# FasterDecoding/TEAL

Hardware: AMD Instinct MI355X
Metric: decode tokens/sec (bs=1), Llama-2-7B fp16 @50% activation sparsity (higher is better)
Workload: dtype f16; 1 GPU; Llama-2-7B bs=1 decode, uniform 50% sparsity, hipGraph-captured step; mode=engine, parallelism=single GPU, context_positions=6..866

## Files before the change

### include/teal_hip.h

```cpp
#ifndef TEAL_HIP_H
#define TEAL_HIP_H

#include <stddef.h>
#include <stdint.h>

#ifdef __cplusplus
extern "C" {
#endif

#define TEAL_OK 0
#define TEAL_ERR_ARG (-1)
#define TEAL_ERR_DTYPE (-2)
#define TEAL_ERR_SHAPE (-3)
#define TEAL_ERR_ALIGN (-4)
#define TEAL_ERR_WORKSPACE (-5)
#define TEAL_ERR_LAUNCH (-6)
#define TEAL_ERR_NO_DEVICE (-7)
#define TEAL_ERR_CONFIG (-8)

#define TEAL_F16 0
#define TEAL_BF16 1

int teal_version(void);
const char* teal_strerror(int code);
// ... 225 lines not shown
#define TEAL_STOP_SEQ 32
#define TEAL_STOP_WORDS 96
#define TEAL_STOP_MAX_IDS 16
#define TEAL_STOP_MAX_SEQS 8
#define TEAL_STOP_MAX_SEQ_LEN 8
#define TEAL_FINISH_RUNNING 0
#define TEAL_FINISH_STOP_TOKEN 1
#define TEAL_FINISH_STOP_SEQUENCE 2
#define TEAL_FINISH_LENGTH 3
#define TEAL_FINISH_CACHE 4
int teal_batched_retire_stops(int32_t* slot_state, const int32_t* tokens, int32_t* pos, const int32_t* history, int history_stride,
                              int32_t* stops, int B, int slot_mask, int max_seq, int count_step, void* stream);


int teal_kv_copy_rows(const void* src_table, const void* dst_table, int n_tensors, int n_heads, int rows, int row_bytes,
                      size_t src_head_stride, size_t dst_head_stride, void* stream);


int teal_cmp_flag_gemv(const void* x, const void* wT, int ld, float* y32, unsigned char* flags, float tau, int Z, int N,
                       int dtype, void* stream);

#ifdef TEAL_DIAGNOSTICS

int teal_set_tuning(int lanes_per_row, int waves, int split, int unroll);

int teal_set_wave_local(int on);

const char* teal_last_launch_desc(void);

int teal_set_fast(int on);

int teal_set_phase_buffer(void* dev_u64);
int teal_set_phase_stride(size_t u64_per_launch);
#endif


int teal_get_config(int Z, int N, int nseg, int* out);

int teal_decode_attention_split_plan(int n_head, int n_kv_head, int head_dim, int max_seq, int nsplit, int roped, int* out);

#ifdef __cplusplus
}
#endif
#endif
```

### teal_amd/_lib.py

```python
from __future__ import annotations

import concurrent.futures
import contextlib
import ctypes
import glob
import os
import shutil
import subprocess
import sys

_PKG = os.path.dirname(os.path.abspath(__file__))
_ROOT = os.path.dirname(_PKG)
CSRC = os.path.join(_PKG, "csrc")
SOURCES = ("teal_kernels.hip", "teal_attention.hip", "teal_sampler.hip", "teal_gemv_w16_f16.hip", "teal_gemv_w16_bf16.hip",
           "teal_gemv_w8_f16.hip", "teal_gemv_w8_bf16.hip", "teal_gemv_fast_f16.hip", "teal_gemv_fast_bf16.hip", "teal_gemv_int4.hip",
           "teal_gemv_fast_w8_f16.hip", "teal_gemv_fast_w8_bf16.hip", "teal_comparators.hip", "teal_prefill.hip",
           "teal_speculative.hip", "teal_batched.hip", "teal_prefix.hip", "teal_logprob.hip", "teal_logit_adjust.hip",
           "teal_sample_rows.hip", "teal_stop.hip")
PRELOAD = {"teal_gemv_fast_f16.hip": 12, "teal_gemv_fast_bf16.hip": 12, "teal_gemv_fast_w8_f16.hip": 12,
           "teal_gemv_fast_w8_bf16.hip": 12, "teal_attention.hip": 12, "teal_sampler.hip": 12}
NO_PACKED_FP32 = ["-Xclang", "-target-feature", "-Xclang", "-packed-fp32-ops"]
FP_CONTRACT = "-ffp-contract=on"
INCLUDE = os.path.join(_ROOT, "include")
OBJ_DIR = os.path.join(CSRC, "_obj")
LIB_PATH = os.path.join(_PKG, "libteal_hip.so")
DIAG_LIB_PATH = os.path.join(_PKG, "libteal_hip_diag.so")
LIB_OVERRIDE = os.environ.get("TEAL_LIB_PATH") or None
OPTIONAL_WITH_OVERRIDE = ("teal_decode_attention_split_roped", "teal_prefill_gemm", "teal_prefill_resid_norm", "teal_prefill_attention",
                          "teal_verify_attention_ws_bytes", "teal_verify_attention", "teal_spec_accept_scratch_bytes", "teal_spec_accept",
                          "teal_batched_sparse_gemm", "teal_batched_round_rows", "teal_batched_decode_attention_ws_bytes",
                          "teal_batched_decode_attention", "teal_batched_sparse_gemm_slots", "teal_batched_decode_attention_slots",
                          "teal_batched_retire", "teal_sample_topk_slot", "teal_kv_copy_rows", "teal_decode_attention_split_plan",
                          "teal_token_logprobs", "teal_score_step", "teal_logit_adjust", "teal_sample_rows",
                          "teal_batched_retire_stops")

EXPORTS = (
    "teal_version", "teal_strerror", "teal_init", "teal_workspace_bytes", "teal_compact",
    "teal_sparse_gemv", "teal_sparse_qkv_gemv", "teal_dense_gemv", "teal_sparse_gateup_silu",
    "teal_get_config", "teal_fused_gemv", "teal_decode_attention", "teal_sample_topk", "teal_sparse_qkv_gemv_ld", "teal_decode_attention_masked", "teal_decode_attention_split", "teal_sparse_qkv_gemv_i8", "teal_decode_attention_split_slabs", "teal_sparse_qkv_gemv_i4",
    "teal_workspace_init", "teal_workspace_release", "teal_sample_topk_ws", "teal_decode_attention_split_ws", "teal_cmp_flag_gemv",
    "teal_decode_attention_split_roped",
    "teal_prefill_gemm", "teal_prefill_resid_norm", "teal_prefill_attention",
    "teal_verify_attention_ws_bytes", "teal_verify_attention", "teal_spec_accept_scratch_bytes", "teal_spec_accept",
    "teal_batched_sparse_gemm", "teal_batched_round_rows", "teal_batched_decode_attention_ws_bytes", "teal_batched_decode_attention",
    "teal_batched_sparse_gemm_slots", "teal_batched_decode_attention_slots", "teal_batched_retire", "teal_sample_topk_slot",
    "teal_kv_copy_rows", "teal_decode_attention_split_plan", "teal_token_logprobs", "teal_score_step",
    "teal_logit_adjust", "teal_sample_rows", "teal_batched_retire_stops",
)

DIAG_EXPORTS = ("teal_set_tuning", "teal_set_fast", "teal_set_wave_local", "teal_set_phase_buffer", "teal_set_phase_stride",
                "teal_last_launch_desc")

_lib = None
_diag = None


def _hipcc() -> str:
    for cand in (os.environ.get("HIPCC"), shutil.which("hipcc"), "/opt/rocm/bin/hipcc"):
        if cand and os.path.exists(cand):
            return cand
    raise RuntimeError("hipcc not found: cannot build libteal_hip.so (no CPU fallback exists)")


def _plan(lib_path: str, obj_dir: str, flags, force: bool, srcs, headers):
    newest_header = max(os.path.getmtime(h) for h in headers)
    hipcc = _hipcc()
    jobs, objs = [], []
    for src in srcs:
        obj = os.path.join(obj_dir, os.path.basename(src)[:-4] + ".o")
        objs.append(obj)
        if not force and os.path.exists(obj) and os.path.getmtime(obj) >= max(os.path.getmtime(src), newest_header):
            continue
        extra = []
        if os.path.basename(src) in PRELOAD:
            extra = ["-mllvm", f"-amdgpu-kernarg-preload-count={PRELOAD[os.path.basename(src)]}"]
        jobs.append(([hipcc, *flags, *extra, "-c", src, "-o", obj], obj))
    return jobs, objs


def build(force: bool = False, verbose: bool = False, out: str | None = None, extra_flags=(), diag: bool = True) -> str:
    headers = glob.glob(os.path.join(CSRC, "*.h")) + [os.path.join(INCLUDE, "teal_hip.h")]
    srcs = [os.path.join(CSRC, f) for f in SOURCES]
    base = ["--offload-arch=gfx950", "-O3", "-std=c++17", "-fPIC", "-Wno-pass-failed", f"-I{INCLUDE}", f"-I{CSRC}", *NO_PACKED_FP32, FP_CONTRACT]
    if out is not None:
# ... 88 lines not shown
        L.teal_batched_round_rows.argtypes = [vp, ci, ci, ci, vp, ci, vp]
        L.teal_batched_decode_attention_ws_bytes.argtypes = [ci, ci, ci]
        L.teal_batched_decode_attention_ws_bytes.restype = sz
        L.teal_batched_decode_attention.argtypes = [vp, ci, vp, vp, vp, vp, vp, vp, sz, ci, ci, ci, ci, ci, ci, vp]
    if hasattr(L, "teal_batched_retire"):
        L.teal_batched_sparse_gemm_slots.argtypes = [vp, vp, vp, ci, ci, vp, ci, ci, vp, sz, ci, ci, vp, vp, ci, ctypes.POINTER(ci), vp]
        L.teal_batched_decode_attention_slots.argtypes = [vp, ci, vp, vp, vp, vp, vp, vp, vp, sz, ci, ci, ci, ci, ci, ci, vp]
        L.teal_batched_retire.argtypes = [vp, vp, vp, ci, ci, ci, ci, vp]
        L.teal_sample_topk_slot.argtypes = [vp, ci, ci, ci, cf, vp, vp, vp, vp, ci, vp, sz, vp, ci, vp]
    if hasattr(L, "teal_kv_copy_rows"):
        L.teal_kv_copy_rows.argtypes = [vp, vp, ci, ci, ci, ci, sz, sz, vp]
    if hasattr(L, "teal_token_logprobs"):
        L.teal_token_logprobs.argtypes = [vp, sz, ci, ci, ci, vp, vp, vp, ci, ci, vp, vp, vp, ci, vp]
        L.teal_score_step.argtypes = [vp, ci, ci, vp, ci, vp, vp, vp, vp]
    if hasattr(L, "teal_logit_adjust"):
        L.teal_logit_adjust.argtypes = [vp, sz, ci, ci, ci, vp, ci, vp, vp, vp, vp, sz, vp, ci, vp]
    if hasattr(L, "teal_sample_rows"):
        L.teal_sample_rows.argtypes = [vp, sz, ci, ci, ci, vp, vp, vp, vp, vp, ci, vp, vp, ci, vp]
    if hasattr(L, "teal_batched_retire_stops"):
        L.teal_batched_retire_stops.argtypes = [vp, vp, vp, vp, ci, vp, ci, ci, ci, ci, vp]
    for name in EXPORTS + (DIAG_EXPORTS if diag else ()):
        if LIB_OVERRIDE and name in OPTIONAL_WITH_OVERRIDE and not hasattr(L, name):
            continue
        getattr(L, name)
        if getattr(L, name).restype is None:
            getattr(L, name).restype = ci
    if diag:
        L.teal_set_tuning.argtypes = [ci, ci, ci, ci]
        L.teal_set_phase_buffer.argtypes = [vp]
        L.teal_set_phase_stride.argtypes = [sz]
        L.teal_set_wave_local.argtypes = [ci]
        L.teal_set_fast.argtypes = [ci]
        L.teal_last_launch_desc.restype = ctypes.c_char_p
    L.teal_is_diagnostics_build = diag
    return L


def load() -> ctypes.CDLL:
    global _lib
    if _lib is None:
        if os.environ.get("TEAL_LIB_FLAVOR", "") == "diag" and not LIB_OVERRIDE:
            _lib = load_diag()
        else:
            _lib = _open(LIB_OVERRIDE or LIB_PATH, False)
    return _lib


def load_diag() -> ctypes.CDLL:
    global _diag
    if _diag is None:
        _diag = _open(DIAG_LIB_PATH, True)
    return _diag


@contextlib.contextmanager
def diagnostics():
    global _lib
    from . import runtime
    prev = load()
    D = load_diag()
    runtime.drop_workspaces()
    _lib = D
    try:
        yield D
    finally:
        D.teal_set_tuning(0, 0, 0, 0)
# ... 13 lines not shown
```

### teal_amd/csrc/teal_attention.hip

```cpp
#include "teal_common.h"

namespace teal {

constexpr int kPhaseRowA = 32;

template <bool BF16, int NT, int HD>
__global__ __launch_bounds__(NT) void decode_attention_kernel(
    const uint16_t* __restrict__ qkv, const uint16_t* __restrict__ rope, const int* __restrict__ pos_ptr,
    uint16_t* __restrict__ k_cache, uint16_t* __restrict__ v_cache, uint16_t* __restrict__ y,
    unsigned long long* __restrict__ mask_out, const float mask_tau,
    const int n_head, const int n_kv, const int max_seq, const float scale, unsigned long long* __restrict__ phase) {
    constexpr int NW = NT / 64;
    constexpr int hd = HD;
    auto stamp_a = [&](const int i) { if (phase && threadIdx.x == 0) phase[(size_t)blockIdx.x * 8 + i] = wall_clock64(); };
    stamp_a(0);
    constexpr int SL = HD / 8;
    constexpr int RW = 64 / SL;
    constexpr int VPF = 256 / (NW * RW) > 0 ? 256 / (NW * RW) : 1;
    extern __shared__ __align__(16) unsigned char smem[];
    float* qs = reinterpret_cast<float*>(smem);
    float* kn = qs + hd;
    float* vn = kn + hd;
    float* red = vn + hd;
    float* part = red + 2 * NW;
// ... 373 lines not shown
#pragma unroll
    for (int w = 0; w < NW; ++w) tot += red[NW + w];
    float o[8];
#pragma unroll
    for (int j = 0; j < 8; ++j) o[j] = 0.0f;
    auto pv_row = [&](const int i, const u32x4 w) {
        const int t = row_of(i);
        if (t >= n) return;
        const float pr = sc[i * STEP + rbase];
        if (!ROPED && t == pos) {
#pragma unroll
            for (int j = 0; j < 8; ++j) o[j] += pr * vn[ds * 8 + j];
        } else {
#pragma unroll
            for (int j = 0; j < 4; ++j) {
                o[2 * j] += pr * bits_to_float(w[j] & 0xFFFFu, BF16);
                o[2 * j + 1] += pr * bits_to_float(w[j] >> 16, BF16);
            }
        }
    };
    if (!rolling) {
#pragma unroll
        for (int i = 0; i < PF; ++i)
            if (i < nsteps) pv_row(i, vreg[i]);
    } else {
        for (int i0 = 0; i0 < nsteps; i0 += RD) {
#pragma unroll
            for (int u = 0; u < RD; ++u) {
                if (i0 + u < nsteps) pv_row(i0 + u, vreg[u]);
                vreg[u] = v_roll(i0 + u + RD);
            }
        }
    }
#pragma unroll
    for (int j = 0; j < 8; ++j) {
        if constexpr (SL <= 8) o[j] = xor_add<8>(o[j]);
        o[j] = xor_add<32>(xor_add<16>(o[j]));
    }
    if (lane < SL) {
#pragma unroll
        for (int j = 0; j < 8; ++j) part[wave * hd + lane * 8 + j] = o[j];
    }
    __syncthreads();
    stamp_p(5);
    if (tid < hd) {
        float acc = 0.0f;
#pragma unroll
        for (int w = 0; w < NW; ++w) acc += part[w * hd + tid];
        out[2 + tid] = acc;
    }
    if (tid == 0) { out[0] = mx; out[1] = tot; }
    stamp_p(7);
}

template <int CTRL>
__device__ __forceinline__ float dpp_lane(const float v) {
    return __builtin_bit_cast(float, __builtin_amdgcn_update_dpp(0, __builtin_bit_cast(int, v), CTRL, 0xf, 0xf, false));
}

template <int NV, int CTRL, int BIT>
__device__ __forceinline__ void fold_level(float* a, const int lane) {
    if constexpr (NV > 1) {
        const bool hi = (lane & BIT) != 0;
#pragma unroll
        for (int k = 0; k < NV / 2; ++k) {
            const float keep = hi ? a[NV / 2 + k] : a[k];
            const float send = hi ? a[k] : a[NV / 2 + k];
            a[k] = keep + dpp_lane<CTRL>(send);
        }
    } else {
        a[0] += dpp_lane<CTRL>(a[0]);
    }
}

template <int REP, int SL>
__device__ __forceinline__ float gqa_reduce_scatter(float* a, const int lane) {
    constexpr int N8 = REP, N4 = (SL == 16 && N8 > 1) ? N8 / 2 : N8, N2 = N4 > 1 ? N4 / 2 : N4, N1 = N2 > 1 ? N2 / 2 : N2;
    static_assert((N1 > 1 ? N1 / 2 : N1) == 1, "more heads than lanes per row");
    if constexpr (SL == 16) fold_level<N8, 0x128, 8>(a, lane);
    fold_level<N4, 0x141, 4>(a, lane);
    fold_level<N2, 0x4E, 2>(a, lane);
    fold_level<N1, 0xB1, 1>(a, lane);
// ... 197 lines not shown
            if (t == pos) w = vnw;
            f32x2 vf[4];
#pragma unroll
            for (int j = 0; j < 4; ++j) vf[j] = (f32x2){bits_to_float(w[j] & 0xFFFFu, BF16), bits_to_float(w[j] >> 16, BF16)};
            float pr[REP];
            const f32x4* pp = reinterpret_cast<const f32x4*>(sc + (size_t)(i * STEP + rbase) * REP);
#pragma unroll
            for (int q4 = 0; q4 < REP / 4; ++q4) {
                const f32x4 pv = pp[q4];
#pragma unroll
                for (int e = 0; e < 4; ++e) pr[q4 * 4 + e] = pv[e];
            }
#pragma unroll
            for (int r = 0; r < REP; ++r) {
                const f32x2 p2 = (f32x2){pr[r], pr[r]};
#pragma unroll
                for (int j = 0; j < 4; ++j) o[r][j] += p2 * vf[j];
            }
        }
    };
    if (nsteps <= PF) {
#pragma unroll
        for (int u = 0; u < PF; ++u)
            if (u < nsteps) v_step(u, vb[u]);
    } else {
        for (int i0 = 0; i0 < nsteps; i0 += RD) {
#pragma unroll
            for (int u = 0; u < RD; ++u) {
                if (i0 + u < nsteps) v_step(i0 + u, vb[u]);
                vb[u] = v_roll(i0 + u + RD);
            }
        }
    }
#pragma unroll
    for (int r = 0; r < REP; ++r)
#pragma unroll
        for (int j = 0; j < 4; ++j)
#pragma unroll
            for (int e = 0; e < 2; ++e) {
                float v = o[r][j][e];
                if constexpr (SL <= 8) v = xor_add<8>(v);
                v = xor_add<32>(xor_add<16>(v));
                o[r][j][e] = v;
            }
    __syncthreads();
    float* part = sc;
    if (lane < SL) {
#pragma unroll
        for (int r = 0; r < REP; ++r)
#pragma unroll
            for (int j = 0; j < 4; ++j)
                *reinterpret_cast<f32x2*>(part + (wave * REP + r) * hd + lane * 8 + 2 * j) = o[r][j];
    }
    __syncthreads();
    for (int c = tid; c < REP * hd; c += NT) {
        float acc = 0.0f;
#pragma unroll
        for (int w = 0; w < NW; ++w) acc += part[w * REP * hd + c];
        out_of(c / hd)[2 + (c % hd)] = acc;
    }
    if (tid < REP) {
        float tot = 0.0f;
#pragma unroll
        for (int w = 0; w < NW; ++w) tot += red[(REP + tid) * NW + w];
        float m = red[tid * NW];
#pragma unroll
        for (int w = 1; w < NW; ++w) m = fmaxf(m, red[tid * NW + w]);
        out_of(tid)[0] = m;
        out_of(tid)[1] = tot;
    }
}

template <bool BF16>
__global__ __launch_bounds__(128) void decode_attention_merge_kernel(const float* __restrict__ partials,
                                                                     uint16_t* __restrict__ y,
                                                                     unsigned long long* __restrict__ mask_out,
                                                                     const float mask_tau, const int hd, const int nsplit) {
    const int h = blockIdx.x, tid = threadIdx.x;
    if (tid >= hd) return;
    merge_head<BF16>(partials + (size_t)h * nsplit * (hd + 2), y + (size_t)h * hd,
                            mask_out ? mask_out + ((size_t)h * hd >> 6) : nullptr, mask_tau, hd, nsplit, tid, tid & 63);
}

constexpr int kGqaMinSeq8 = 2048;
constexpr int kGqaMinSeq = 4096;
constexpr size_t kGqaMaxLds = 128 * 1024;
constexpr size_t kSplitMaxLds = 64 * 1024;

inline bool split_shape_ok(const int n_head, const int n_kv_head, const int head_dim, const int max_seq, const int nsplit) {
    return (head_dim == 64 || head_dim == 128) && n_head > 0 && n_kv_head > 0 && n_head % n_kv_head == 0 && max_seq > 0 &&
           nsplit >= 1 && nsplit <= 64;
// ... 186 lines not shown
```

### teal_amd/csrc/teal_common.h

```cpp
#pragma once
#include <hip/hip_runtime.h>

#include <math.h>
#include <stdint.h>

#include <type_traits>

#include "teal_hip.h"

namespace teal {


typedef uint32_t u32x4 __attribute__((ext_vector_type(4)));
typedef uint32_t u32x2 __attribute__((ext_vector_type(2)));
typedef _Float16 f16x2 __attribute__((ext_vector_type(2)));

constexpr int kMaxSeg = 3;
constexpr int kMaxSplit = 32;


struct Seg {
    const void* w;
    void* y;
    float tau;
// ... 155 lines not shown
    const int t0 = __builtin_amdgcn_readlane(v, 15);
    const int t1 = __builtin_amdgcn_readlane(v, 31);
    const int t2 = __builtin_amdgcn_readlane(v, 47);
    return v + (lane >= 16 ? t0 : 0) + (lane >= 32 ? t1 : 0) + (lane >= 48 ? t2 : 0);
}

__device__ __forceinline__ float wave_sum_f(float v) {
    auto shr = [](float a, auto ctrl) {
        return __builtin_bit_cast(float, __builtin_amdgcn_update_dpp(0, __builtin_bit_cast(int, a), decltype(ctrl)::value, 0xf, 0xf, false));
    };
    v += shr(v, std::integral_constant<int, 0x111>{});
    v += shr(v, std::integral_constant<int, 0x112>{});
    v += shr(v, std::integral_constant<int, 0x114>{});
    v += shr(v, std::integral_constant<int, 0x118>{});
    const int iv = __builtin_bit_cast(int, v);
    return __builtin_bit_cast(float, __builtin_amdgcn_readlane(iv, 15)) +
           __builtin_bit_cast(float, __builtin_amdgcn_readlane(iv, 31)) +
           __builtin_bit_cast(float, __builtin_amdgcn_readlane(iv, 47)) +
           __builtin_bit_cast(float, __builtin_amdgcn_readlane(iv, 63));
}

template <int OFF>
__device__ __forceinline__ float xor_add(const float v) {
    const int iv = __builtin_bit_cast(int, v);
    if constexpr (OFF == 8) {
        return v + __builtin_bit_cast(float, __builtin_amdgcn_update_dpp(iv, iv, 0x128, 0xf, 0xf, false));
    } else if constexpr (OFF == 16) {
        return v + __builtin_bit_cast(float, __builtin_amdgcn_ds_swizzle(iv, 0x401F));
    } else {
        return v + __shfl_xor(v, OFF);
    }
}

__device__ __forceinline__ float wave_max_f(float v) {
    auto shr = [](float a, auto ctrl) {
        return __builtin_bit_cast(float, __builtin_amdgcn_update_dpp(__builtin_bit_cast(int, a), __builtin_bit_cast(int, a), decltype(ctrl)::value, 0xf, 0xf, false));
    };
    v = fmaxf(v, shr(v, std::integral_constant<int, 0x111>{}));
    v = fmaxf(v, shr(v, std::integral_constant<int, 0x112>{}));
    v = fmaxf(v, shr(v, std::integral_constant<int, 0x114>{}));
    v = fmaxf(v, shr(v, std::integral_constant<int, 0x118>{}));
    const int iv = __builtin_bit_cast(int, v);
    return fmaxf(fmaxf(__builtin_bit_cast(float, __builtin_amdgcn_readlane(iv, 15)), __builtin_bit_cast(float, __builtin_amdgcn_readlane(iv, 31))),
                 fmaxf(__builtin_bit_cast(float, __builtin_amdgcn_readlane(iv, 47)), __builtin_bit_cast(float, __builtin_amdgcn_readlane(iv, 63))));
}

template <int SL>
__device__ __forceinline__ float row_slices_sum(float v) {
    if constexpr (SL == 16) {
        auto ror = [](float a, auto ctrl) {
            return __builtin_bit_cast(float, __builtin_amdgcn_update_dpp(0, __builtin_bit_cast(int, a), decltype(ctrl)::value, 0xf, 0xf, false));
        };
        v += ror(v, std::integral_constant<int, 0x128>{});
        v += ror(v, std::integral_constant<int, 0x124>{});
        v += ror(v, std::integral_constant<int, 0x122>{});
        v += ror(v, std::integral_constant<int, 0x121>{});
        return v;
    } else {
#pragma unroll
        for (int d = 1; d < SL; d <<= 1) v += __shfl_xor(v, d);
        return v;
    }
}


__device__ __forceinline__ int lane_rank(unsigned long long mask) {
// ... 41 lines not shown
```

### teal_amd/csrc/teal_gemv_fast.h

```cpp
#pragma once
#include "teal_gemv_fast_decl.h"
#include "teal_gemv_kernel.h"

namespace teal {

#define TEAL_FAST_ARGS_BATCH(a)                                                                                         \
    asm volatile("" ::"s"((a).w0), "s"((a).w1), "s"((a).y), "s"((a).ws), "s"((a).mask_out), "s"((a).resid_out),          \
                 "s"((a).phase), "s"((a).ticket), "s"((a).ld0), "s"((a).ld1), "s"((a).seg_tile1), "s"((a).seg_tile2), "s"((a).tau0),       \
                 "s"((a).tau1), "s"((a).tau2), "s"((a).mask_tau), "s"((a).ws_stride), "s"((a).att_hd), "s"((a).att_ns),  \
                 "s"((a).cap), "s"((a).w1_tile), "s"((a).scale0), "s"((a).scale1), "s"((a).sum32))


template <bool BF16, int MODE, bool PAIR, int LPR, int KR, bool EXACT, bool PHASE, int U = 4, bool W8 = false, bool ROPE = false>
__global__ __launch_bounds__(1024) void gemv_fast_kernel(const void* in0, const void* in1, const void* in2,
                                                         const int* row_index, const int Z, const int nslabs,
                                                         const float eps, const int split_p, const FastArgs a) {
    static_assert(!(W8 && PAIR), "int8 gate|up runs unpaired (two images of 128-byte row segments)");
    static_assert(!ROPE || (MODE == 1 && !PAIR && !W8), "the RoPE / KV-append epilogue belongs to the fused wqkv projection");
    constexpr int WAVES = 16;
    constexpr int RPW = 64 / LPR;
    constexpr int CPL = 8;
    constexpr int BN = LPR * CPL;
    constexpr int WB = W8 ? 1 : 2;
    using wvec = std::conditional_t<W8, u32x2, u32x4>;
// ... 315 lines not shown
            consume(wa, w2a, xa);
            if constexpr (PHASE) { if (!first_done) { first_done = true; stamp(4); } }
            eb = ebn;
            if (!fb) break;
            ebn = eb + STEP;
            fa = full(ebn);
            if (fa) issue(wa, w2a, xa, ebn);
            consume(wbb, w2b, xb);
            eb = ebn;
        }
        if (eb < nloc) {
#pragma unroll
            for (int u = 0; u < U; ++u) {
                const int e = eb + u * RPW + g;
                const bool ok = e < nloc;
                const uint32_t ent = list[ok ? e : nloc - 1];
                xa[u] = ok ? bits_to_float(ent & 0xFFFFu, BF16) : 0.0f;
                wvec t = __builtin_nontemporal_load(reinterpret_cast<const wvec*>(wp + (size_t)(ent >> 16) * ldb));
                if (!ok) t = wvec(0u);
                wa[u] = t;
                if constexpr (PAIR) {
                    wvec t2 = __builtin_nontemporal_load(reinterpret_cast<const wvec*>(wp2 + (size_t)(ent >> 16) * ldb2));
                    if (!ok) t2 = wvec(0u);
                    w2a[u] = t2;
                }
            }
            consume(wa, w2a, xa);
        }
    }
    stamp(5);
    if (prio_set) __builtin_amdgcn_s_setprio(0);
    if constexpr (PHASE) { if (a.phase && lane == 0) a.phase[(size_t)bid * kPhaseRow + 16 + wave] = wall_clock64(); }

#pragma unroll
    for (int j = 0; j < CPL; ++j) {
        if constexpr (LPR <= 8) acc[j] = xor_add<8>(acc[j]);
        acc[j] = xor_add<32>(xor_add<16>(acc[j]));
    }
    if constexpr (PAIR) {
#pragma unroll
        for (int j = 0; j < 8; ++j) {
            if constexpr (LPR <= 8) acc2[j] = xor_add<8>(acc2[j]);
            acc2[j] = xor_add<32>(xor_add<16>(acc2[j]));
        }
    }
    if (lane < LPR) {
        float* r = red + wave * BN + lane * CPL;
#pragma unroll
        for (int j = 0; j < CPL; ++j) r[j] = acc[j];
        if constexpr (PAIR) {
            float* r2 = red + (WAVES + wave) * BN + lane * 8;
#pragma unroll
            for (int j = 0; j < 8; ++j) r2[j] = acc2[j];
        }
    }
    float* xsw = red + (PAIR ? 2 : 1) * WAVES * BN;
    if constexpr (W8) {
        if constexpr (LPR <= 8) xs = xor_add<8>(xs);
        xs = xor_add<32>(xor_add<16>(xs));
        if (lane == 0) xsw[wave] = xs;
    }
    __syncthreads();
    stamp(6);
    if (tid < BN) {
        const uint32_t c = (uint32_t)tile * BN + tid;
        float gs = 0.0f, us = 0.0f;
#pragma unroll
        for (int wv = 0; wv < WAVES; ++wv) {
            gs += red[wv * BN + tid];
            if constexpr (PAIR) us += red[(WAVES + wv) * BN + tid];
        }
        if constexpr (W8) {
            float bias = 0.0f;
#pragma unroll
            for (int wv = 0; wv < WAVES; ++wv) bias += xsw[wv];
            bias *= kInt8Bias;
            gs = (gs - bias) * bits_to_float(scb, BF16);
        }
        if constexpr (PAIR) {
            const float g16 = bits_to_float(float_to_bits<BF16>(gs), BF16);
            const float u16 = bits_to_float(float_to_bits<BF16>(us), BF16);
            const float sl = bits_to_float(float_to_bits<BF16>(g16 / (1.0f + expf(-g16))), BF16);
            const uint32_t hb = float_to_bits<BF16>(sl * u16);
            reinterpret_cast<uint16_t*>(a.y)[c] = (uint16_t)hb;
            const float hv = bits_to_float(hb, BF16);
            const unsigned long long mko = __ballot(keep_rule(hv, a.mask_tau) || (hv != hv));
            if (a.mask_out && lane == 0) a.mask_out[c >> 6] = mko;
        } else if (a.ws_stride == 0) {
            if constexpr (ROPE) {
                const uint16_t b16 = float_to_bits<BF16>(gs);
                const float f = bits_to_float(b16, BF16);
                const float pr = __shfl_xor(f, 1);
                const float cs = bits_to_float(rope_cs & 0xFFFFu, BF16), sn = bits_to_float(rope_cs >> 16, BF16);
                const uint16_t rb = float_to_bits<BF16>((tid & 1) ? rope_odd(pr, f, cs, sn) : rope_even(f, pr, cs, sn));
                const uint32_t dimq = (uint32_t)a.rope_dim, kvw = (uint32_t)a.rope_kv, hdm = (uint32_t)a.rope_hd;
                if (c < dimq) {
                    reinterpret_cast<uint16_t*>(a.y)[c] = rb;
                } else {
                    const bool isk = c < dimq + kvw;
                    const uint32_t cc = c - dimq - (isk ? 0u : kvw);
                    const uint32_t kvh = cc / hdm, d = cc & (hdm - 1u);
                    (isk ? a.kc : a.vc)[((size_t)kvh * (size_t)a.rope_max_seq + (size_t)rope_p) * hdm + d] = isk ? rb : b16;
                }
            } else if (a.act0 && s == 0) {
                reinterpret_cast<uint16_t*>(a.y)[c] = silu_bits<BF16>(gs);
            } else if (a.sum32) {
                reinterpret_cast<float*>(a.y)[c] = gs;
            } else {
                reinterpret_cast<uint16_t*>(a.y)[c] = float_to_bits<BF16>(gs);
            }
        } else if (!a.ticket) {
            a.ws[c * (uint32_t)a.ws_stride + slice] = gs;
        } else {
            __hip_atomic_store(&a.ws[c * (uint32_t)a.ws_stride + slice], gs, __ATOMIC_RELAXED, __HIP_MEMORY_SCOPE_AGENT);
        }
    }
    if constexpr (!PAIR) {
        if (a.ticket) {
            float* tflag = reinterpret_cast<float*>(smem);
            asm volatile("s_waitcnt vmcnt(0)" ::: "memory");
            __syncthreads();
            if (tid == 0) {
                const unsigned t = __hip_atomic_fetch_add(&a.ticket[tile], 1u, __ATOMIC_RELAXED, __HIP_MEMORY_SCOPE_AGENT);
                tflag[0] = (t == (unsigned)split - 1u) ? 1.0f : 0.0f;
            }
            __syncthreads();
            if (tflag[0] != 0.0f && tid < BN) {
                const uint32_t c = (uint32_t)tile * BN + tid;
                float sum = 0.0f;
                for (int sl = 0; sl < split; ++sl)
                    sum += __hip_atomic_load(&a.ws[c * (uint32_t)a.ws_stride + sl], __ATOMIC_RELAXED, __HIP_MEMORY_SCOPE_AGENT);
                if (a.sum32) reinterpret_cast<float*>(a.y)[c] = sum;
                else reinterpret_cast<uint16_t*>(a.y)[c] = (a.act0 && s == 0) ? silu_bits<BF16>(sum) : float_to_bits<BF16>(sum);
                if (tid == 0) __hip_atomic_store(&a.ticket[tile], 0u, __ATOMIC_RELAXED, __HIP_MEMORY_SCOPE_AGENT);
            }
        }
// ... 110 lines not shown
```

### teal_amd/csrc/teal_gemv_kernel.h

```cpp
#pragma once
#include "teal_common.h"

#pragma clang fp contract(off)

namespace teal {

template <bool BF16>
__device__ __forceinline__ void fma8(float (&acc)[8], const u32x4 w, const float xv) {
#pragma unroll
    for (int j = 0; j < 4; ++j) {
        const uint32_t q = w[j];
        float lo, hi;
        if (BF16) {
            lo = __uint_as_float(q << 16);
            hi = __uint_as_float(q & 0xFFFF0000u);
        } else {
            const f16x2 h = __builtin_bit_cast(f16x2, q);
            lo = (float)h.x;
            hi = (float)h.y;
        }
        acc[2 * j] = fmaf(lo, xv, acc[2 * j]);
        acc[2 * j + 1] = fmaf(hi, xv, acc[2 * j + 1]);
    }
}
// ... 438 lines not shown
            if (p.phase && !first_done) { first_done = true; stamp(p, 4); }
            eb = ebn;
            if (!fb) break;
            ebn = eb + STEP;
            fa = full(ebn);
            if (fa) issue(wa, w2a, xa, ebn);
            consume(wb, w2b, xb);
            eb = ebn;
        }
        if (eb < nloc) {
#pragma unroll
            for (int u = 0; u < U; ++u) {
                const int e = eb + u * estride + g;
                const bool ok = e < nloc;
                const uint32_t ent = lp[ok ? e : nloc - 1];
                xa[u] = ok ? bits_to_float(ent & 0xFFFFu, BF16) : 0.0f;
                wvec t = __builtin_nontemporal_load(
                    reinterpret_cast<const wvec*>(wp + (size_t)(ent >> 16) * ldb));
                if (!W8 && !ok) t = wvec(0u);
                wa[u] = t;
                if constexpr (PAIR) {
                    wvec t2 = __builtin_nontemporal_load(
                        reinterpret_cast<const wvec*>(wp2 + (size_t)(ent >> 16) * ldb2));
                    if (!W8 && !ok) t2 = wvec(0u);
                    w2a[u] = t2;
                }
            }
            consume(wa, w2a, xa);
        }
    }

    stamp(p, 5);
    if (p.phase && lane == 0) p.phase[(size_t)blockIdx.x * kPhaseRow + 16 + (wave & 15)] = wall_clock64();
#pragma unroll
    for (int off = LPR; off < 64; off <<= 1) {
#pragma unroll
        for (int j = 0; j < 8; ++j) acc[j] += __shfl_xor(acc[j], off);
        if constexpr (PAIR) {
#pragma unroll
            for (int j = 0; j < 8; ++j) acc2[j] += __shfl_xor(acc2[j], off);
        }
    }
    if (lane < LPR) {
        float* r = red + wave * BN + lane * 8;
#pragma unroll
        for (int j = 0; j < 8; ++j) r[j] = acc[j];
        if constexpr (PAIR) {
            float* r2 = red + (WAVES + wave) * BN + lane * 8;
#pragma unroll
            for (int j = 0; j < 8; ++j) r2[j] = acc2[j];
        }
    }
    float* xsw = red + (PAIR ? 2 : 1) * WAVES * BN;
    if constexpr (W8) {
#pragma unroll
        for (int off = LPR; off < 64; off <<= 1) {
            xs += __shfl_xor(xs, off);
            if constexpr (PAIR) xs2 += __shfl_xor(xs2, off);
        }
        if (lane == 0) {
            xsw[wave] = col_ok ? xs : 0.0f;
            if constexpr (PAIR) xsw[WAVES + wave] = col_ok ? xs2 : 0.0f;
        }
    }
    __syncthreads();
    stamp(p, 6);
    float bias = 0.0f, bias2 = 0.0f;
    if constexpr (W8) {
#pragma unroll
        for (int wv = 0; wv < WAVES; ++wv) {
            bias += xsw[wv];
            if constexpr (PAIR) bias2 += xsw[WAVES + wv];
        }
        bias *= kInt8Bias;
        bias2 *= kInt8Bias;
    }
    if constexpr (PAIR) {
        static_assert(!PAIR || BN <= WAVES * 64, "one thread per tile column");
        if (tid < BN) {
            const int c = tcol0 + tid;
            uint32_t hb = 0u;
            bool kp = false;
            if (c < sg.ncols) {
// ... 118 lines not shown
```

### teal_amd/csrc/teal_kernels.hip

```cpp
#include "teal_common.h"
#include "teal_gemv_fast_decl.h"

#include <limits.h>
#include <stdio.h>
#include <stdlib.h>

#include <mutex>
#include <vector>

namespace teal {

template <int WAVES, bool BF16>
__device__ __forceinline__ void wg_ballot_prefix(const uint16_t* __restrict__ x, const int Z,
                                                 const float tau, const bool nan_keeps,
                                                 unsigned long long* masks, int* prefix) {
    const int lane = threadIdx.x & 63;
    const int wave = threadIdx.x >> 6;
    const int nch = (Z + 63) >> 6;
    for (int c = wave; c < nch; c += WAVES) {
        const int m = (c << 6) + lane;
        bool k = false;
        if (m < Z) {
            const float v = bits_to_float(x[m], BF16);
            k = keep_rule(v, tau) || (nan_keeps && (v != v));
// ... 38 lines not shown
__global__ __launch_bounds__(256) void gateup_silu_epilogue_kernel(const Params p, void* h) {
    const int n = blockIdx.x * 256 + threadIdx.x;
    const int N = p.seg[0].ncols;
    if (n >= N) return;
    float g = 0.0f, u = 0.0f;
    for (int k = 0; k < p.split; ++k) {
        g += p.ws[(size_t)k * p.ws_ld + n];
        u += p.ws[(size_t)k * p.ws_ld + N + n];
    }
    const float g16 = bits_to_float(float_to_bits<BF16>(g), BF16);
    const float u16 = bits_to_float(float_to_bits<BF16>(u), BF16);
    const float sl = g16 / (1.0f + expf(-g16));
    const float sl16 = bits_to_float(float_to_bits<BF16>(sl), BF16);
    reinterpret_cast<uint16_t*>(h)[n] = float_to_bits<BF16>(sl16 * u16);
}

template <bool BF16>
__global__ __launch_bounds__(1024) void compact_kernel(const uint16_t* __restrict__ x, const int Z,
                                                       const float tau, int32_t* __restrict__ idx_out,
                                                       int32_t* __restrict__ count_out) {
    extern __shared__ __align__(16) unsigned char smem[];
    const int nch = (Z + 63) >> 6;
    unsigned long long* masks = reinterpret_cast<unsigned long long*>(smem);
    int* prefix = reinterpret_cast<int*>(masks + nch);
    wg_ballot_prefix<16, BF16>(x, Z, tau, false, masks, prefix);
    const int lane = threadIdx.x & 63;
    const int wave = threadIdx.x >> 6;
    for (int c = wave; c < nch; c += 16) {
        const unsigned long long mask = masks[c];
        if ((mask >> lane) & 1ull) idx_out[prefix[c] + lane_rank(mask)] = (c << 6) + lane;
    }
    if (threadIdx.x == 0) *count_out = prefix[nch];
}




#ifdef TEAL_DIAGNOSTICS
Config g_override = {0, 0, 0, 0};
unsigned long long* g_phase = nullptr;
size_t g_phase_stride = 0;
int g_phase_seq = 0;
int g_wave_local = 1;
int g_fast = 1;
char g_last_desc[160] = "";
#endif

constexpr int kMaxDevices = 64;
static DeviceCtx g_dev[kMaxDevices] = {};
static std::mutex g_dev_mu;

DeviceCtx* device_ctx() {
    int dev = 0;
    if (hipGetDevice(&dev) != hipSuccess) { (void)hipGetLastError(); return nullptr; }
    if (dev < 0 || dev >= kMaxDevices) return nullptr;
    DeviceCtx* c = &g_dev[dev];
    if (c->num_cu > 0) return c;
    std::lock_guard<std::mutex> lk(g_dev_mu);
    if (c->num_cu > 0) return c;
    int cu = 0;
    if (hipDeviceGetAttribute(&cu, hipDeviceAttributeMultiprocessorCount, dev) != hipSuccess || cu <= 0) {
        (void)hipGetLastError();
        return nullptr;
    }
    c->gqa_lds_ok = attention_device_init();
    c->num_cu = cu;
// ... 419 lines not shown
    auto in = [](int v, std::initializer_list<int> ok) {
        for (int o : ok) if (v == o) return true;
        return false;
    };
    if (!in(lanes_per_row, {0, 8, 16, 32, 64}) || !in(waves, {0, 16}) ||
        !in(unroll, {0, 4}) || split < 0 || split > kMaxSplit)
        return TEAL_ERR_CONFIG;
    g_override = {lanes_per_row, waves, split, unroll};
    return TEAL_OK;
}

const char* teal_last_launch_desc(void) { return g_last_desc; }

int teal_set_fast(int on) {
    g_fast = on ? 1 : 0;
    return TEAL_OK;
}

int teal_set_wave_local(int on) {
    g_wave_local = on ? 1 : 0;
    return TEAL_OK;
}

int teal_set_phase_buffer(void* dev_u64) {
    g_phase = reinterpret_cast<unsigned long long*>(dev_u64);
    g_phase_seq = 0;
    return TEAL_OK;
}

int teal_set_phase_stride(size_t u64_per_launch) {
    g_phase_stride = u64_per_launch;
    g_phase_seq = 0;
    return TEAL_OK;
}
#endif

int teal_get_config(int Z, int N, int nseg, int* out) {
    if (!out || Z <= 0 || N <= 0) return TEAL_ERR_ARG;
    const Config c = pick_config(Z, N, nseg);
    out[0] = c.lpr;
    out[1] = c.waves;
    out[2] = c.split;
    out[3] = c.unroll;
    out[4] = ((N + c.lpr * 8 - 1) / (c.lpr * 8)) * c.split;
    return TEAL_OK;
}

int teal_compact(const void* x, float tau, int Z, int dtype, int32_t* idx_out, int32_t* count_out,
                 void* stream) {
    if (!x || !idx_out || !count_out || Z <= 0) return TEAL_ERR_ARG;
    if (dtype != TEAL_F16 && dtype != TEAL_BF16) return TEAL_ERR_DTYPE;
    if (Z > 65536) return TEAL_ERR_SHAPE;
    const int nch = (Z + 63) >> 6;
    const size_t lds = (size_t)nch * 8 + (size_t)(nch + 2) * 4;
    hipStream_t st = reinterpret_cast<hipStream_t>(stream);
    const uint16_t* xp = reinterpret_cast<const uint16_t*>(x);
    if (dtype == TEAL_BF16)
        hipLaunchKernelGGL((compact_kernel<true>), dim3(1), dim3(1024), lds, st, xp, Z, tau, idx_out, count_out);
    else
        hipLaunchKernelGGL((compact_kernel<false>), dim3(1), dim3(1024), lds, st, xp, Z, tau, idx_out, count_out);
    return hipGetLastError() == hipSuccess ? TEAL_OK : TEAL_ERR_LAUNCH;
}

int teal_sparse_qkv_gemv(const void* x, const void* wT, void* y, float tau_q, float tau_k,
                         float tau_v, int Z, int N, int N_q, int N_kv, int dtype, void* ws,
                         size_t ws_bytes, void* stream) {
// ... 227 lines not shown
```

Baseline: 548.6 tokens/s.

## Replace cross-lane shuffle reductions with permlane swap reduce-scatter in GEMV and attention

Replaces the per-accumulator xor-shuffle butterfly reduction (xor 16/32 on each of 8 values) with a reduce-scatter built on permlane16/permlane32 swap instructions, so each lane ends up owning two reduced columns instead of all lanes holding all eight. The LDS partial-sum layout changes to a swizzled slot mapping, and the final cross-wave sum loads all wave partials before adding. The fast GEMV's RoPE epilogue precomputes destination pointers and cos/sin before the barrier and uses DPP for the neighbour exchange. A diagnostic probe kernel compares the new reduction against the shuffle version. The change cuts cross-lane instruction count but adds index arithmetic and a layout that must match across writers and readers.

```diff
diff --git a/include/teal_hip.h b/include/teal_hip.h
--- a/include/teal_hip.h
+++ b/include/teal_hip.h
@@ -281,6 +281,8 @@
 
 int teal_set_phase_buffer(void* dev_u64);
 int teal_set_phase_stride(size_t u64_per_launch);
+
+int teal_probe_row_reduce(const void* in_u32, void* scatter_u32, void* shuffle_u32, int nwaves, int lanes_per_row, void* stream);
 #endif
 
 
diff --git a/teal_amd/_lib.py b/teal_amd/_lib.py
--- a/teal_amd/_lib.py
+++ b/teal_amd/_lib.py
@@ -49,7 +49,7 @@
 )
 
 DIAG_EXPORTS = ("teal_set_tuning", "teal_set_fast", "teal_set_wave_local", "teal_set_phase_buffer", "teal_set_phase_stride",
-                "teal_last_launch_desc")
+                "teal_last_launch_desc", "teal_probe_row_reduce")
 
 _lib = None
 _diag = None
@@ -204,6 +204,7 @@
         L.teal_set_wave_local.argtypes = [ci]
         L.teal_set_fast.argtypes = [ci]
         L.teal_last_launch_desc.restype = ctypes.c_char_p
+        L.teal_probe_row_reduce.argtypes = [vp, vp, vp, ci, ci, vp]
     L.teal_is_diagnostics_build = diag
     return L
 
diff --git a/teal_amd/csrc/teal_attention.hip b/teal_amd/csrc/teal_attention.hip
--- a/teal_amd/csrc/teal_attention.hip
+++ b/teal_amd/csrc/teal_attention.hip
@@ -429,22 +429,26 @@
             }
         }
     }
-#pragma unroll
-    for (int j = 0; j < 8; ++j) {
-        if constexpr (SL <= 8) o[j] = xor_add<8>(o[j]);
-        o[j] = xor_add<32>(xor_add<16>(o[j]));
-    }
-    if (lane < SL) {
-#pragma unroll
-        for (int j = 0; j < 8; ++j) part[wave * hd + lane * 8 + j] = o[j];
-    }
+    float olo, ohi;
+    row_reduce_scatter<SL>(o, olo, ohi);
+    if (SL == 16 || (lane & 15) < SL) {
+        const int slot = scatter_slot((lane & 15) * 8 + (lane >> 4));
+        part[wave * hd + slot] = olo;
+        part[wave * hd + (slot ^ 4)] = ohi;
+    }
+    int pidx = scatter_slot(tid & (hd - 1)), oidx = 2 + (tid & (hd - 1));
+    asm volatile("" : "+v"(pidx), "+v"(oidx));
     __syncthreads();
     stamp_p(5);
     if (tid < hd) {
+        float pw[NW];
+#pragma unroll
+        for (int w = 0; w < NW; ++w) pw[w] = part[w * hd + pidx];
+        __builtin_amdgcn_sched_barrier(0);
         float acc = 0.0f;
 #pragma unroll
-        for (int w = 0; w < NW; ++w) acc += part[w * hd + tid];
-        out[2 + tid] = acc;
+        for (int w = 0; w < NW; ++w) acc += pw[w];
+        out[oidx] = acc;
     }
     if (tid == 0) { out[0] = mx; out[1] = tot; }
     stamp_p(7);
@@ -708,31 +712,32 @@
             }
         }
     }
-#pragma unroll
-    for (int r = 0; r < REP; ++r)
-#pragma unroll
-        for (int j = 0; j < 4; ++j)
-#pragma unroll
-            for (int e = 0; e < 2; ++e) {
-                float v = o[r][j][e];
-                if constexpr (SL <= 8) v = xor_add<8>(v);
-                v = xor_add<32>(xor_add<16>(v));
-                o[r][j][e] = v;
-            }
+    float olo[REP], ohi[REP];
+#pragma unroll
+    for (int r = 0; r < REP; ++r) {
+        const float v[8] = {o[r][0][0], o[r][0][1], o[r][1][0], o[r][1][1], o[r][2][0], o[r][2][1], o[r][3][0], o[r][3][1]};
+        row_reduce_scatter<SL>(v, olo[r], ohi[r]);
+    }
     __syncthreads();
     float* part = sc;
-    if (lane < SL) {
-#pragma unroll
-        for (int r = 0; r < REP; ++r)
-#pragma unroll
-            for (int j = 0; j < 4; ++j)
-                *reinterpret_cast<f32x2*>(part + (wave * REP + r) * hd + lane * 8 + 2 * j) = o[r][j];
+    if (SL == 16 || (lane & 15) < SL) {
+        const int slot = scatter_slot((lane & 15) * 8 + (lane >> 4));
+#pragma unroll
+        for (int r = 0; r < REP; ++r) {
+            part[(wave * REP + r) * hd + slot] = olo[r];
+            part[(wave * REP + r) * hd + (slot ^ 4)] = ohi[r];
+        }
     }
     __syncthreads();
     for (int c = tid; c < REP * hd; c += NT) {
+        const float* psrc = part + (c & ~(hd - 1)) + scatter_slot(c & (hd - 1));
+        float pw[NW];
+#pragma unroll
+        for (int w = 0; w < NW; ++w) pw[w] = psrc[w * REP * hd];
+        __builtin_amdgcn_sched_barrier(0);
         float acc = 0.0f;
 #pragma unroll
-        for (int w = 0; w < NW; ++w) acc += part[w * REP * hd + c];
+        for (int w = 0; w < NW; ++w) acc += pw[w];
         out_of(c / hd)[2 + (c % hd)] = acc;
     }
     if (tid < REP) {
diff --git a/teal_amd/csrc/teal_common.h b/teal_amd/csrc/teal_common.h
--- a/teal_amd/csrc/teal_common.h
+++ b/teal_amd/csrc/teal_common.h
@@ -211,6 +211,27 @@
     }
 }
 
+__device__ __forceinline__ float swap16_add(const float a, const float b) {
+    const auto r = __builtin_amdgcn_permlane16_swap(__builtin_bit_cast(unsigned, a), __builtin_bit_cast(unsigned, b), false, false);
+    return __builtin_bit_cast(float, (unsigned)r[0]) + __builtin_bit_cast(float, (unsigned)r[1]);
+}
+__device__ __forceinline__ float swap32_add(const float a, const float b) {
+    const auto r = __builtin_amdgcn_permlane32_swap(__builtin_bit_cast(unsigned, a), __builtin_bit_cast(unsigned, b), false, false);
+    return __builtin_bit_cast(float, (unsigned)r[0]) + __builtin_bit_cast(float, (unsigned)r[1]);
+}
+
+template <int LPR>
+__device__ __forceinline__ void row_reduce_scatter(const float (&v)[8], float& lo, float& hi) {
+    static_assert(LPR == 8 || LPR == 16, "row groups of 8 or 16 lanes");
+    float t[8];
+#pragma unroll
+    for (int j = 0; j < 8; ++j) t[j] = LPR <= 8 ? xor_add<8>(v[j]) : v[j];
+    lo = swap32_add(swap16_add(t[0], t[1]), swap16_add(t[2], t[3]));
+    hi = swap32_add(swap16_add(t[4], t[5]), swap16_add(t[6], t[7]));
+}
+
+__device__ __forceinline__ int scatter_slot(const int c) { return c ^ ((c >> 4) & 4); }
+
 __device__ __forceinline__ float wave_max_f(float v) {
     auto shr = [](float a, auto ctrl) {
         return __builtin_bit_cast(float, __builtin_amdgcn_update_dpp(__builtin_bit_cast(int, a), __builtin_bit_cast(int, a), decltype(ctrl)::value, 0xf, 0xf, false));
diff --git a/teal_amd/csrc/teal_gemv_fast.h b/teal_amd/csrc/teal_gemv_fast.h
--- a/teal_amd/csrc/teal_gemv_fast.h
+++ b/teal_amd/csrc/teal_gemv_fast.h
@@ -371,26 +371,18 @@
     if (prio_set) __builtin_amdgcn_s_setprio(0);
     if constexpr (PHASE) { if (a.phase && lane == 0) a.phase[(size_t)bid * kPhaseRow + 16 + wave] = wall_clock64(); }
 
-#pragma unroll
-    for (int j = 0; j < CPL; ++j) {
-        if constexpr (LPR <= 8) acc[j] = xor_add<8>(acc[j]);
-        acc[j] = xor_add<32>(xor_add<16>(acc[j]));
-    }
-    if constexpr (PAIR) {
-#pragma unroll
-        for (int j = 0; j < 8; ++j) {
-            if constexpr (LPR <= 8) acc2[j] = xor_add<8>(acc2[j]);
-            acc2[j] = xor_add<32>(xor_add<16>(acc2[j]));
-        }
-    }
-    if (lane < LPR) {
-        float* r = red + wave * BN + lane * CPL;
-#pragma unroll
-        for (int j = 0; j < CPL; ++j) r[j] = acc[j];
+    float lo, hi, lo2 = 0.0f, hi2 = 0.0f;
+    row_reduce_scatter<LPR>(acc, lo, hi);
+    if constexpr (PAIR) row_reduce_scatter<LPR>(acc2, lo2, hi2);
+    if (LPR == 16 || (lane & 15) < LPR) {
+        const int slot = scatter_slot((lane & 15) * CPL + (lane >> 4));
+        float* r = red + wave * BN;
+        r[slot] = lo;
+        r[slot ^ 4] = hi;
         if constexpr (PAIR) {
-            float* r2 = red + (WAVES + wave) * BN + lane * 8;
-#pragma unroll
-            for (int j = 0; j < 8; ++j) r2[j] = acc2[j];
+            float* r2 = red + (WAVES + wave) * BN;
+            r2[slot] = lo2;
+            r2[slot ^ 4] = hi2;
         }
     }
     float* xsw = red + (PAIR ? 2 : 1) * WAVES * BN;
@@ -399,15 +391,49 @@
         xs = xor_add<32>(xor_add<16>(xs));
         if (lane == 0) xsw[wave] = xs;
     }
+    float rope_c = 0.0f, rope_s = 0.0f;
+    uint16_t* rope_dst = nullptr;
+    bool rope_rot = false;
+    if constexpr (ROPE) {
+        if (tid < BN) {
+            const uint32_t c = (uint32_t)tile * BN + tid;
+            rope_c = bits_to_float(rope_cs & 0xFFFFu, BF16);
+            rope_s = bits_to_float(rope_cs >> 16, BF16);
+            const uint32_t dimq = (uint32_t)a.rope_dim, kvw = (uint32_t)a.rope_kv, hdm = (uint32_t)a.rope_hd;
+            const bool isq = c < dimq, isk = c < dimq + kvw;
+            const uint32_t cc = c - dimq - (isk ? 0u : kvw);
+            const uint32_t kvh = cc >> (6u + (hdm >> 7)), d = cc & (hdm - 1u);
+            rope_rot = isk;
+            rope_dst = isq ? reinterpret_cast<uint16_t*>(a.y) + c
+                           : (isk ? a.kc : a.vc) + ((size_t)kvh * (size_t)a.rope_max_seq + (size_t)rope_p) * hdm + d;
+            asm volatile("" : "+v"(rope_dst), "+v"(rope_c), "+v"(rope_s));
+        }
+    }
     __syncthreads();
     stamp(6);
     if (tid < BN) {
         const uint32_t c = (uint32_t)tile * BN + tid;
+        const float* rsrc = red + scatter_slot(tid);
         float gs = 0.0f, us = 0.0f;
-#pragma unroll
-        for (int wv = 0; wv < WAVES; ++wv) {
-            gs += red[wv * BN + tid];
-            if constexpr (PAIR) us += red[(WAVES + wv) * BN + tid];
+        if constexpr (KR <= 8) {
+            float pg[WAVES], pu[PAIR ? WAVES : 1];
+#pragma unroll
+            for (int wv = 0; wv < WAVES; ++wv) {
+                pg[wv] = rsrc[wv * BN];
+                if constexpr (PAIR) pu[wv] = rsrc[(WAVES + wv) * BN];
+            }
+            __builtin_amdgcn_sched_barrier(0);
+#pragma unroll
+            for (int wv = 0; wv < WAVES; ++wv) {
+                gs += pg[wv];
+                if constexpr (PAIR) us += pu[wv];
+            }
+        } else {
+#pragma unroll
+            for (int wv = 0; wv < WAVES; ++wv) {
+                gs += rsrc[wv * BN];
+                if constexpr (PAIR) us += rsrc[(WAVES + wv) * BN];
+            }
         }
         if constexpr (W8) {
             float bias = 0.0f;
@@ -429,18 +455,9 @@
             if constexpr (ROPE) {
                 const uint16_t b16 = float_to_bits<BF16>(gs);
                 const float f = bits_to_float(b16, BF16);
-                const float pr = __shfl_xor(f, 1);
-                const float cs = bits_to_float(rope_cs & 0xFFFFu, BF16), sn = bits_to_float(rope_cs >> 16, BF16);
-                const uint16_t rb = float_to_bits<BF16>((tid & 1) ? rope_odd(pr, f, cs, sn) : rope_even(f, pr, cs, sn));
-                const uint32_t dimq = (uint32_t)a.rope_dim, kvw = (uint32_t)a.rope_kv, hdm = (uint32_t)a.rope_hd;
-                if (c < dimq) {
-                    reinterpret_cast<uint16_t*>(a.y)[c] = rb;
-                } else {
-                    const bool isk = c < dimq + kvw;
-                    const uint32_t cc = c - dimq - (isk ? 0u : kvw);
-                    const uint32_t kvh = cc / hdm, d = cc & (hdm - 1u);
-                    (isk ? a.kc : a.vc)[((size_t)kvh * (size_t)a.rope_max_seq + (size_t)rope_p) * hdm + d] = isk ? rb : b16;
-                }
+                const float pr = __builtin_bit_cast(float, __builtin_amdgcn_update_dpp(0, __builtin_bit_cast(int, f), 0xB1, 0xf, 0xf, false));
+                const uint16_t rb = float_to_bits<BF16>((tid & 1) ? rope_odd(pr, f, rope_c, rope_s) : rope_even(f, pr, rope_c, rope_s));
+                *(__attribute__((address_space(1))) uint16_t*)rope_dst = rope_rot ? rb : b16;
             } else if (a.act0 && s == 0) {
                 reinterpret_cast<uint16_t*>(a.y)[c] = silu_bits<BF16>(gs);
             } else if (a.sum32) {
diff --git a/teal_amd/csrc/teal_gemv_kernel.h b/teal_amd/csrc/teal_gemv_kernel.h
--- a/teal_amd/csrc/teal_gemv_kernel.h
+++ b/teal_amd/csrc/teal_gemv_kernel.h
@@ -494,23 +494,40 @@
 
     stamp(p, 5);
     if (p.phase && lane == 0) p.phase[(size_t)blockIdx.x * kPhaseRow + 16 + (wave & 15)] = wall_clock64();
-#pragma unroll
-    for (int off = LPR; off < 64; off <<= 1) {
-#pragma unroll
-        for (int j = 0; j < 8; ++j) acc[j] += __shfl_xor(acc[j], off);
+    if constexpr (LPR <= 16) {
+        float lo, hi;
+        row_reduce_scatter<LPR>(acc, lo, hi);
+        const int c0 = (lane & 15) * 8 + (lane >> 4);
+        if (LPR == 16 || (lane & 15) < LPR) {
+            red[wave * BN + c0] = lo;
+            red[wave * BN + c0 + 4] = hi;
+        }
         if constexpr (PAIR) {
-#pragma unroll
-            for (int j = 0; j < 8; ++j) acc2[j] += __shfl_xor(acc2[j], off);
-        }
-    }
-    if (lane < LPR) {
-        float* r = red + wave * BN + lane * 8;
-#pragma unroll
-        for (int j = 0; j < 8; ++j) r[j] = acc[j];
-        if constexpr (PAIR) {
-            float* r2 = red + (WAVES + wave) * BN + lane * 8;
-#pragma unroll
-            for (int j = 0; j < 8; ++j) r2[j] = acc2[j];
+            row_reduce_scatter<LPR>(acc2, lo, hi);
+            if (LPR == 16 || (lane & 15) < LPR) {
+                red[(WAVES + wave) * BN + c0] = lo;
+                red[(WAVES + wave) * BN + c0 + 4] = hi;
+            }
+        }
+    } else {
+#pragma unroll
+        for (int off = LPR; off < 64; off <<= 1) {
+#pragma unroll
+            for (int j = 0; j < 8; ++j) acc[j] += __shfl_xor(acc[j], off);
+            if constexpr (PAIR) {
+#pragma unroll
+                for (int j = 0; j < 8; ++j) acc2[j] += __shfl_xor(acc2[j], off);
+            }
+        }
+        if (lane < LPR) {
+            float* r = red + wave * BN + lane * 8;
+#pragma unroll
+            for (int j = 0; j < 8; ++j) r[j] = acc[j];
+            if constexpr (PAIR) {
+                float* r2 = red + (WAVES + wave) * BN + lane * 8;
+#pragma unroll
+                for (int j = 0; j < 8; ++j) r2[j] = acc2[j];
+            }
         }
     }
     float* xsw = red + (PAIR ? 2 : 1) * WAVES * BN;
diff --git a/teal_amd/csrc/teal_kernels.hip b/teal_amd/csrc/teal_kernels.hip
--- a/teal_amd/csrc/teal_kernels.hip
+++ b/teal_amd/csrc/teal_kernels.hip
@@ -94,6 +94,30 @@
     }
     if (threadIdx.x == 0) *count_out = prefix[nch];
 }
+
+
+#ifdef TEAL_DIAGNOSTICS
+template <int LPR>
+__global__ __launch_bounds__(64) void row_reduce_probe_kernel(const uint32_t* __restrict__ in, uint32_t* __restrict__ scatter_out,
+                                                              uint32_t* __restrict__ shuffle_out) {
+    const int lane = threadIdx.x;
+    const size_t base = ((size_t)blockIdx.x * 64 + lane) * 8;
+    float v[8], b[8];
+#pragma unroll
+    for (int j = 0; j < 8; ++j) v[j] = b[j] = __builtin_bit_cast(float, in[base + j]);
+    float lo, hi;
+    row_reduce_scatter<LPR>(v, lo, hi);
+    scatter_out[((size_t)blockIdx.x * 64 + lane) * 2] = __builtin_bit_cast(uint32_t, lo);
+    scatter_out[((size_t)blockIdx.x * 64 + lane) * 2 + 1] = __builtin_bit_cast(uint32_t, hi);
+#pragma unroll
+    for (int off = LPR; off < 64; off <<= 1) {
+#pragma unroll
+        for (int j = 0; j < 8; ++j) b[j] += __shfl_xor(b[j], off);
+    }
+#pragma unroll
+    for (int j = 0; j < 8; ++j) shuffle_out[base + j] = __builtin_bit_cast(uint32_t, b[j]);
+}
+#endif
 
 
 
@@ -579,6 +603,17 @@
     g_phase_stride = u64_per_launch;
     g_phase_seq = 0;
     return TEAL_OK;
+}
+
+int teal_probe_row_reduce(const void* in_u32, void* scatter_u32, void* shuffle_u32, int nwaves, int lanes_per_row, void* stream) {
+    if (!in_u32 || !scatter_u32 || !shuffle_u32 || nwaves <= 0 || (lanes_per_row != 8 && lanes_per_row != 16)) return TEAL_ERR_ARG;
+    const uint32_t* in = reinterpret_cast<const uint32_t*>(in_u32);
+    uint32_t* so = reinterpret_cast<uint32_t*>(scatter_u32);
+    uint32_t* sh = reinterpret_cast<uint32_t*>(shuffle_u32);
+    hipStream_t st = reinterpret_cast<hipStream_t>(stream);
+    if (lanes_per_row == 8) hipLaunchKernelGGL((row_reduce_probe_kernel<8>), dim3(nwaves), dim3(64), 0, st, in, so, sh);
+    else hipLaunchKernelGGL((row_reduce_probe_kernel<16>), dim3(nwaves), dim3(64), 0, st, in, so, sh);
+    return hipGetLastError() == hipSuccess ? TEAL_OK : TEAL_ERR_LAUNCH;
 }
 #endif
 
```

Result: faster. 559.7 tokens/s (median of 6 runs) (+2.0%).
